# irconde/SSL4POLYP

Hardware: AMD Instinct MI355X
Metric: training-step images/sec/node, ViT-B/16 224^2 (cls fine-tune) (higher is better)
Workload: dtype bf16; 1 GPU; ViT-B/16 classification fine-tune, bs=64/GPU, 224^2, AdamW, random init, finetune mode full (finetune.py:49-91); global_batch=64, parallelism=dp1, launch=eager, lr_schedule=constant

## Files before the change

include/polypmae.h:

```cpp
#ifndef POLYPMAE_H
#define POLYPMAE_H
#include <stddef.h>
#include <stdint.h>

#ifdef __cplusplus
extern "C" {
#endif

enum pm_status { PM_OK = 0, PM_EINVAL = -1, PM_ESHAPE = -2, PM_EARCH = -3, PM_ELAUNCH = -4, PM_EALIGN = -5 };
enum pm_dtype { PM_F32 = 0, PM_BF16 = 1, PM_F16 = 2 };

enum pm_epilogue {
  PM_EPI_STORE = 0,
  PM_EPI_GELU = 1,
  PM_EPI_RESIDUAL = 2,
  PM_EPI_DGELU = 3,
  PM_EPI_ACCUM = 4
};

const char* pm_strerror(int status);
int pm_abi_version(void);

int pm_layernorm_fwd(const float* x, long ldx, const float* gamma, const float* beta, void* y, int out_dtype,
                     float* mean, float* rstd, int M, int D, float eps, void* stream);
// ... 21 lines not shown

#define PM_GEMM_GENERIC 0
#define PM_GEMM_LDS128 1
#define PM_GEMM_RING 2
#define PM_GEMM_RING_WGRAD 3
typedef struct pm_gemm_plan_info {
  int family;
  int cfg;
  int tile_m, tile_n;
  int split_k;
  int band;
  size_t ws_bytes;
} pm_gemm_plan_info;
int pm_gemm_plan(int a_kmajor, int b_kmajor, int in_dtype, int has_bias, int c_dtype, int ldc_is_n, int epilogue, int M, int N,
                 int K, size_t ws_bytes, const pm_gemm_opts* opts, pm_gemm_plan_info* info);

typedef struct pm_wgrad_item {
  const void* dY;
  long lddy;
  const void* X;
  long ldx;
  float* dW;
  long lddw;
  int n_out, n_in;
  int accumulate;
  float* dbias;
} pm_wgrad_item;
#define PM_GROUP_WHOLE_K (-1)
int pm_wgrad_group(const pm_wgrad_item* items, int n, int K, int in_dtype, int max_blocks, void* workspace, size_t ws_bytes,
                   void* stream);
// ... 253 lines not shown
```

ssl4polyp_amd/_lib.py:

```python
from __future__ import annotations

import ctypes
import os
from ctypes import c_char_p, c_float, c_int, c_long, c_void_p

PM_F32, PM_BF16, PM_F16 = 0, 1, 2
EPI_STORE, EPI_GELU, EPI_RESIDUAL, EPI_DGELU, EPI_ACCUM = 0, 1, 2, 3, 4

_HERE = os.path.dirname(os.path.abspath(__file__))
LIB_PATH = os.environ.get("POLYPMAE_LIB") or os.path.join(_HERE, "lib", "libpolypmae.so")

P, I, L, F = c_void_p, c_int, c_long, c_float

SIGNATURES = {
    "pm_layernorm_fwd": [P, L, P, P, P, I, P, P, I, I, F, P],
    "pm_layernorm_bwd": [P, I, P, L, P, P, P, P, L, P, L, P, I, P, P, P, I, I, P, ctypes.c_size_t, P],
    "pm_vit_block_fwd": [P, P],
    "pm_vit_block_bwd": [P, P],
    "pm_gemm": [P, L, I, P, L, I, I, P, P, L, I, I, P, P, I, I, I, P],
    "pm_gemm_ws": [P, L, I, P, L, I, I, P, P, L, I, I, P, P, I, I, I, P, ctypes.c_size_t, P],
    "pm_gemm_ex": [P, L, I, P, L, I, I, P, P, L, I, I, P, P, I, I, I, P, ctypes.c_size_t, P, P],
    "pm_wgrad_group": [P, I, I, I, I, P, ctypes.c_size_t, P],
    "pm_wgrad_group_plan": [P, I, I, I, P, P, P],
    "pm_gemm_plan": [I, I, I, I, I, I, I, I, I, I, ctypes.c_size_t, P, P],
    "pm_attention_plan": [I, I, I, I, I, I, P],
    "pm_attention_fwd": [P, P, P, I, I, I, I, I, P],
    "pm_attention_bwd": [P, P, P, P, P, P, I, I, I, I, I, P],
    "pm_colsum": [P, L, I, P, I, I, P],
    "pm_colsum_ws": [P, L, I, P, I, I, P, ctypes.c_size_t, P],
    "pm_patch_im2col": [P, P, P, L, I, I, I, I, I, I, P],
    "pm_pad_cast": [P, L, P, L, I, I, I, I, I, P],
    "pm_unpad_add": [P, L, P, L, I, I, I, P],
    "pm_assemble_tokens": [P, P, P, P, P, I, I, I, P],
    "pm_assemble_tokens_bwd": [P, P, P, I, P, P, I, I, I, P],
    "pm_mae_noise": [P, L, ctypes.c_ulonglong, ctypes.c_uint, P],
    "pm_mae_masking": [P, P, P, P, I, I, I, P],
    "pm_mae_unshuffle": [P, P, P, P, P, I, I, I, I, P],
    "pm_mae_unshuffle_bwd": [P, P, P, I, P, I, I, I, I, P, ctypes.c_size_t, P],
    "pm_mae_loss_fwd": [P, P, L, I, P, I, I, I, I, I, P],
# ... 161 lines not shown
```

ssl4polyp_amd/csrc/pm_common.h:

```cpp
#pragma once
#include <hip/hip_runtime.h>
#include <stdint.h>
#include "../../include/polypmae.h"

#ifdef PM_AUTO_VMCNT
#define PM_LDS_IMAGE
#else
#define PM_LDS_IMAGE __restrict__
#endif

#define PM_WAVE 64

typedef __attribute__((ext_vector_type(8))) __bf16 bf16x8;
typedef __attribute__((ext_vector_type(4))) __bf16 bf16x4;
typedef __attribute__((ext_vector_type(2))) __bf16 bf16x2;
typedef __attribute__((ext_vector_type(8))) _Float16 f16x8;
typedef __attribute__((ext_vector_type(4))) _Float16 f16x4;
typedef __attribute__((ext_vector_type(4))) short short4v;
typedef __attribute__((ext_vector_type(16))) float f32x16;
typedef __attribute__((ext_vector_type(4))) float f32x4;
typedef __attribute__((ext_vector_type(2))) float f32x2;
typedef __attribute__((ext_vector_type(4))) unsigned int u32x4;
typedef __attribute__((ext_vector_type(2))) unsigned int u32x2;

// ... 287 lines not shown
  }
#endif
  return gelu_erf4(v);
}
template <typename T> __device__ __forceinline__ f32x4 gelu_act_grad4(f32x4 v) {
#ifdef PM_GELU_POLY
  if constexpr (sizeof(T) == 2) {
    const f32x2 a = gelu_poly_grad2(f32x2{v[0], v[1]}), b = gelu_poly_grad2(f32x2{v[2], v[3]});
    return f32x4{a[0], a[1], b[0], b[1]};
  }
#endif
  return gelu_erf_grad4(v);
}
template <typename T> __device__ __forceinline__ f32x4 round_through(f32x4 v) {
  return f32x4{to_f32<T>(from_f32<T>(v[0])), to_f32<T>(from_f32<T>(v[1])), to_f32<T>(from_f32<T>(v[2])), to_f32<T>(from_f32<T>(v[3]))};
}

constexpr int kF0298 = 2446, kF0390 = 3196, kF0541 = 4433, kF0765 = 6270, kF0899 = 7373, kF1175 = 9633, kF1501 = 12299, kF1847 = 15137,
              kF1961 = 16069, kF2053 = 16819, kF2562 = 20995, kF3072 = 25172;
__device__ __forceinline__ int jdescale(int x, int n) { return (x + (1 << (n - 1))) >> n; }

__device__ __forceinline__ void jidct8(int* c, int s, bool first) {
  int z2 = c[2 * s], z3 = c[6 * s];
  int z1 = (z2 + z3) * kF0541;
  const int e2 = z1 + z3 * (-kF1847), e3 = z1 + z2 * kF0765;
  z2 = c[0];
  z3 = c[4 * s];
  const int e0 = (z2 + z3) << 13, e1 = (z2 - z3) << 13;
  const int t10 = e0 + e3, t13 = e0 - e3, t11 = e1 + e2, t12 = e1 - e2;
  int o0 = c[7 * s], o1 = c[5 * s], o2 = c[3 * s], o3 = c[s];
// ... 78 lines not shown
```

ssl4polyp_amd/csrc/pm_gemm.hip:

```cpp
#include "pm_common.h"
#include <type_traits>

namespace {

constexpr int BM = 128, BN = 128, KB = 128;
constexpr int TILE_BYTES = 128 * KB;
constexpr int kThreads = 256;
constexpr int STAGE_ROW = 64 * 4 + 16;
constexpr int STAGE_BYTES = 64 * STAGE_ROW;
constexpr int GLDS_LDS_BYTES = (4 * STAGE_BYTES > 4 * TILE_BYTES) ? 4 * STAGE_BYTES : 4 * TILE_BYTES;

struct GemmArgs {
  const void* X;
  const void* W;
  long ldx, ldw;
  const float* bias;
  void* C;
  long ldc;
  void* aux;
  const float* resid;
  int M, N, K;
  int epilogue;
  int c_dtype;
  int tiles_m, tiles_n;
  int split_k;
  int ksteps_split;
  float* xsum;
  int xsum_store;
  int col_major;
#ifdef PM_GEMM_STAMP
  unsigned long long* stamps;
#endif
};

#ifdef PM_GEMM_STAMP
#define PM_STAMP(i)                               \
  do {                                            \
    __builtin_amdgcn_sched_barrier(0);            \
    stamp_t[i] = __builtin_readcyclecounter();    \
    __builtin_amdgcn_sched_barrier(0);            \
  } while (0)
#else
#define PM_STAMP(i)
#endif
// ... 138 lines not shown
    } else if (epi == PM_EPI_DGELU) {
      const f32x4 pre = load4<T>(reinterpret_cast<const T*>(a.aux) + off);
      v *= gelu_act_grad4<T>(pre);
    }
    if (a.c_dtype == PM_F32) {
      store4<float>(reinterpret_cast<float*>(a.C) + off, v);
    } else if constexpr (sizeof(T) == 2) {
      store4<T>(reinterpret_cast<T*>(a.C) + off, v);
    } else {
      if (a.c_dtype == PM_F16) store4<_Float16>(reinterpret_cast<_Float16*>(a.C) + off, v);
      else store4<__bf16>(reinterpret_cast<__bf16*>(a.C) + off, v);
    }
  }
}

template <typename E, int NV>
__device__ __forceinline__ void epilogue_batch(const GemmArgs& a, int epi, const long (&off)[NV], const bool (&ok)[NV],
                                               f32x4 (&v)[NV]) {
  if (epi == PM_EPI_RESIDUAL || epi == PM_EPI_ACCUM) {
    const float* src = epi == PM_EPI_RESIDUAL ? a.resid : reinterpret_cast<const float*>(a.C);
    f32x4 r[NV];
#pragma unroll
    for (int e = 0; e < NV; ++e) r[e] = *reinterpret_cast<const f32x4*>(src + off[e]);
#pragma unroll
    for (int e = 0; e < NV; ++e)
      if (ok[e]) *reinterpret_cast<f32x4*>(reinterpret_cast<float*>(a.C) + off[e]) = r[e] + v[e];
    return;
  }
  if (epi == PM_EPI_DGELU) {
    f32x4 pre[NV];
#pragma unroll
    for (int e = 0; e < NV; ++e) pre[e] = load4<E>(reinterpret_cast<const E*>(a.aux) + off[e]);
#pragma unroll
    for (int e = 0; e < NV; ++e) v[e] *= gelu_act_grad4<E>(pre[e]);
  } else if (epi == PM_EPI_GELU) {
#pragma unroll
    for (int e = 0; e < NV; ++e) {
      if (a.aux && ok[e]) store4<E>(reinterpret_cast<E*>(a.aux) + off[e], v[e]);
      v[e] = gelu_act4<E>(round_through<E>(v[e]));
    }
  }
  if (a.c_dtype == PM_F32) {
#pragma unroll
    for (int e = 0; e < NV; ++e)
      if (ok[e]) store4<float>(reinterpret_cast<float*>(a.C) + off[e], v[e]);
  } else {
#pragma unroll
    for (int e = 0; e < NV; ++e)
      if (ok[e]) store4<E>(reinterpret_cast<E*>(a.C) + off[e], v[e]);
  }
}

template <typename E, int NV>
__device__ __forceinline__ void epilogue_batch8(const GemmArgs& a, int epi, const long (&off)[NV], const bool (&ok)[NV],
                                                f32x4 (&lo)[NV], f32x4 (&hi)[NV]) {
  if (epi == PM_EPI_DGELU) {
    f32x4 plo[NV], phi[NV];
#pragma unroll
    for (int u = 0; u < NV; ++u) load8_16<E>(reinterpret_cast<const E*>(a.aux) + off[u], plo[u], phi[u]);
#pragma unroll
    for (int u = 0; u < NV; ++u) {
      lo[u] *= gelu_act_grad4<E>(plo[u]);
      hi[u] *= gelu_act_grad4<E>(phi[u]);
    }
  } else if (epi == PM_EPI_GELU) {
#pragma unroll
    for (int u = 0; u < NV; ++u) {
      if (a.aux && ok[u]) store8_16<E>(reinterpret_cast<E*>(a.aux) + off[u], lo[u], hi[u]);
      lo[u] = gelu_act4<E>(round_through<E>(lo[u]));
      hi[u] = gelu_act4<E>(round_through<E>(hi[u]));
    }
  }
#pragma unroll
  for (int u = 0; u < NV; ++u)
    if (ok[u]) store8_16<E>(reinterpret_cast<E*>(a.C) + off[u], lo[u], hi[u]);
}

__device__ __forceinline__ void swap_halves(float& x, float& y) {
  typedef __attribute__((ext_vector_type(2))) unsigned u32x2;
  const u32x2 r = __builtin_amdgcn_permlane32_swap(__float_as_uint(x), __float_as_uint(y), false, false);
  x = __uint_as_float(r[0]);
  y = __uint_as_float(r[1]);
}

template <typename T, bool XK, bool WK>
// ... 237 lines not shown
  Frag16 f;
  f.u[0] = ((unsigned)(unsigned short)lo[0]) | (((unsigned)(unsigned short)lo[1]) << 16);
  f.u[1] = ((unsigned)(unsigned short)lo[2]) | (((unsigned)(unsigned short)lo[3]) << 16);
  f.u[2] = ((unsigned)(unsigned short)hi[0]) | (((unsigned)(unsigned short)hi[1]) << 16);
  f.u[3] = ((unsigned)(unsigned short)hi[2]) | (((unsigned)(unsigned short)hi[3]) << 16);
  return f;
}

template <int N> __device__ __forceinline__ void wait_vmcnt() {
  if constexpr (N == 0) asm volatile("s_waitcnt vmcnt(0)" ::: "memory");
  else if constexpr (N == 1) asm volatile("s_waitcnt vmcnt(1)" ::: "memory");
  else if constexpr (N == 2) asm volatile("s_waitcnt vmcnt(2)" ::: "memory");
  else if constexpr (N == 3) asm volatile("s_waitcnt vmcnt(3)" ::: "memory");
  else if constexpr (N == 4) asm volatile("s_waitcnt vmcnt(4)" ::: "memory");
  else if constexpr (N == 6) asm volatile("s_waitcnt vmcnt(6)" ::: "memory");
  else if constexpr (N == 8) asm volatile("s_waitcnt vmcnt(8)" ::: "memory");
  else if constexpr (N == 12) asm volatile("s_waitcnt vmcnt(12)" ::: "memory");
  else if constexpr (N == 16) asm volatile("s_waitcnt vmcnt(16)" ::: "memory");
  else if constexpr (N == 24) asm volatile("s_waitcnt vmcnt(24)" ::: "memory");
  else static_assert(N == 0, "add the immediate");
}

template <int BM_, int BN_, bool WK, bool DIRECT, bool PP, bool XK, bool XSUM, typename E>
__device__ __forceinline__ void gemm_v3_tile(GemmArgs& a, const int tile, const int split_idx) {
  constexpr int STAGES = V3_STAGES, NW = V3_WAVES;
  constexpr int WN = BN_ / 64, WM = NW / WN;
  constexpr int TM = BM_ / WM, TN = BN_ / WN;
  constexpr int MT = TM / 32, NTL = TN / 32;
  constexpr int XB = BM_ * 64, WB = BN_ * 64;
  constexpr int SB = XB + WB;
  constexpr int G = (SB / 1024 + NW - 1) / NW;
  static_assert((WB % (1024 * NW)) == 0 && ((XB % (1024 * NW)) == 0 || (!XK && XB == 12288 && DIRECT)),
                "whole wave-instructions per wave, except the 192-row k-normal X tile");
  extern __shared__ __attribute__((aligned(16))) char smem[];
  const int tid = threadIdx.x, lane = tid & 63;
  const int wave = __builtin_amdgcn_readfirstlane(tid >> 6);
  const int wm = wave / WN, wn = wave % WN;
#ifdef PM_GEMM_STAMP
  const unsigned long long stamp_entry = __builtin_readcyclecounter();
  const unsigned long long stamp_entry_rt = __builtin_amdgcn_s_memrealtime();
  unsigned long long stamp_loop_end = 0, stamp_loop_end_rt = 0;
  auto stamp_finish = [&]() {
    const unsigned long long t_issued = __builtin_readcyclecounter();
    asm volatile("s_waitcnt vmcnt(0)" ::: "memory");
    const unsigned long long t_acked = __builtin_readcyclecounter();
    if (a.stamps && lane == 0 && blockIdx.y == 0) {
      unsigned long long* o = a.stamps + ((long)blockIdx.x * NW + wave) * 16;
      o[8] = stamp_entry; o[9] = stamp_loop_end; o[10] = t_issued; o[11] = t_acked;
      o[12] = stamp_entry_rt; o[13] = stamp_loop_end_rt;
    }
  };
#endif
// ... 201 lines not shown
#endif
  } else {
    constexpr int DP = STAGES - 2;
    const int gq = wave >> 2;
#pragma unroll
    for (int t = 0; t < DP; ++t)
      if (t < nk) issue(t);
    constexpr bool UNEVEN = (XB % 8192) != 0;
    auto wait_one_stage_in_flight = [&]() {
      if constexpr (UNEVEN) {
        if (gq == 0) wait_vmcnt<G>(); else wait_vmcnt<G - 1>();
      } else {
        wait_vmcnt<G>();
      }
    };
    if (nk > 1) wait_one_stage_in_flight();
    else wait_vmcnt<0>();
    if (gq == 1) __builtin_amdgcn_s_barrier();
#ifdef PM_GEMM_STAMP
    unsigned long long stamp_t[8], stamp_acc[7] = {0, 0, 0, 0, 0, 0, 0};
#endif
    for (int t = 0; t < nk; ++t) {
      PM_STAMP(0);
      __builtin_amdgcn_s_barrier();
      PM_STAMP(1);
      Frag16 fw[2][NTL], fx[2][MT];
      read_frags(t, fw, fx);
      __builtin_amdgcn_sched_barrier(0);
      PM_STAMP(2);
      if (t + DP < nk) issue(t + DP);
      PM_STAMP(3);
      if (t + 2 < nk) wait_one_stage_in_flight();
      else wait_vmcnt<0>();
      PM_STAMP(4);
      asm volatile("s_waitcnt lgkmcnt(0)" ::: "memory");
      __builtin_amdgcn_sched_barrier(0);
      PM_STAMP(5);
      __builtin_amdgcn_s_barrier();
      PM_STAMP(6);
      mma_all(fw, fx);
#ifdef PM_GEMM_STAMP
      PM_STAMP(7);
#pragma unroll
      for (int i = 0; i < 7; ++i) stamp_acc[i] += stamp_t[i + 1] - stamp_t[i];
#endif
    }
#ifdef PM_GEMM_STAMP
    if (a.stamps && lane == 0 && blockIdx.y == 0) {
#pragma unroll
      for (int i = 0; i < 7; ++i) a.stamps[((long)blockIdx.x * NW + wave) * 16 + i] = stamp_acc[i];
      a.stamps[((long)blockIdx.x * NW + wave) * 16 + 7] = nk;
    }
#endif
    if (gq == 0) __builtin_amdgcn_s_barrier();
  }
#ifdef PM_GEMM_STAMP
  stamp_loop_end = __builtin_readcyclecounter();
  stamp_loop_end_rt = __builtin_amdgcn_s_memrealtime();
#endif
  if constexpr (XSUM) {
    if (do_xsum && lane < 16) {
#pragma unroll
      for (int j = 0; j < MT; ++j) {
        const int m = m0 + wm * TM + 32 * j + lane;
        if (m < a.M) a.xsum[m] = (a.xsum_store ? 0.f : a.xsum[m]) + xs[j][0];
        if (m + 16 < a.M) a.xsum[m + 16] = (a.xsum_store ? 0.f : a.xsum[m + 16]) + xs[j][1];
      }
    }
  }
  const int h = lane >> 5;
  const int epi = a.epilogue;
  if constexpr (DIRECT) {
    if (a.c_dtype != PM_F32 && epi != PM_EPI_RESIDUAL && epi != PM_EPI_ACCUM && (a.N & 7) == 0 && (a.ldc & 7) == 0) {
      constexpr int NV8 = NTL * 2;
      long noff8[NV8];
      bool nok8[NV8];
      f32x4 b0[NV8], b1[NV8];
#pragma unroll
      for (int i = 0; i < NTL; ++i)
#pragma unroll
        for (int p = 0; p < 2; ++p) {
          const int n = n0 + wn * TN + i * 32 + 16 * p + 8 * h;
          nok8[i * 2 + p] = n < a.N;
          noff8[i * 2 + p] = n < a.N ? n : a.N - 8;
        }
#pragma unroll
// ... 67 lines not shown
#pragma unroll
        for (int g = 0; g < 4; ++g) {
          const int e = i * 4 + g;
          off[g] = row + noff[e];
          ok[g] = mok && nok[e];
          v[g] = f32x4{acc[i][j][4 * g], acc[i][j][4 * g + 1], acc[i][j][4 * g + 2], acc[i][j][4 * g + 3]} + bv[e];
        }
        epilogue_batch<E, 4>(a, epi, off, ok, v);
      }
    }
#ifdef PM_GEMM_STAMP
    stamp_finish();
#endif
    return;
  }
  __syncthreads();
  char* st = smem + wave * V3_STAGE_WAVE;
#pragma unroll
  for (int mh = 0; mh < MT / 2; ++mh) {
#pragma unroll
    for (int nh = 0; nh < NTL / 2; ++nh) {
#pragma unroll
      for (int j = 0; j < 2; ++j) {
        const int ml = j * 32 + (lane & 31);
#pragma unroll
        for (int i = 0; i < 2; ++i)
#pragma unroll
          for (int g = 0; g < 4; ++g) {
            const f32x16& t16 = acc[nh * 2 + i][mh * 2 + j];
            const f32x4 v = {t16[4 * g], t16[4 * g + 1], t16[4 * g + 2], t16[4 * g + 3]};
// ... 13 lines not shown
        }
#pragma unroll
        for (int it4 = 0; it4 < 2; ++it4) {
          long off[4];
          bool ok[4];
          f32x4 lo[4], hi[4];
#pragma unroll
          for (int u = 0; u < 4; ++u) {
            const int ml = (it4 * 4 + u) * 8 + (lane >> 3);
            const int m = mw + ml;
            ok[u] = m < a.M && nok8;
            off[u] = (long)(m < a.M ? m : a.M - 1) * a.ldc + ncl8;
            lo[u] = *reinterpret_cast<const f32x4*>(st + ml * STAGE_ROW + c8 * 4) + b0;
            hi[u] = *reinterpret_cast<const f32x4*>(st + ml * STAGE_ROW + c8 * 4 + 16) + b1;
          }
          epilogue_batch8<E, 4>(a, epi, off, ok, lo, hi);
        }
        __builtin_amdgcn_wave_barrier();
        continue;
      }
      const int c4 = (lane & 15) * 4, n = nw + c4;
      const bool nok = n < a.N;
      const long ncl = nok ? n : a.N - 4;
      f32x4 bv = {0.f, 0.f, 0.f, 0.f};
      if (a.bias) bv = *reinterpret_cast<const f32x4*>(a.bias + ncl);
#pragma unroll
      for (int it4 = 0; it4 < 4; ++it4) {
        long off[4];
        bool ok[4];
        f32x4 v[4];
#pragma unroll
        for (int u = 0; u < 4; ++u) {
          const int ml = (it4 * 4 + u) * 4 + (lane >> 4);
          const int m = mw + ml;
          ok[u] = m < a.M && nok;
          off[u] = (long)(m < a.M ? m : a.M - 1) * a.ldc + ncl;
          v[u] = *reinterpret_cast<const f32x4*>(st + ml * STAGE_ROW + c4 * 4) + bv;
        }
        epilogue_batch<E, 4>(a, epi, off, ok, v);
      }
      __builtin_amdgcn_wave_barrier();
    }
  }
#ifdef PM_GEMM_STAMP
  stamp_finish();
#endif
}

template <int BM_, int BN_, bool WK, bool DIRECT, bool PP, bool XK, typename E>
__global__ __launch_bounds__(V3_WAVES * 64, 2) void gemm_v3_kernel(GemmArgs a) {
  gemm_v3_tile<BM_, BN_, WK, DIRECT, PP, XK, false, E>(a, xcd_remap(blockIdx.x, gridDim.x), blockIdx.y);
}

constexpr int kMaxGroup = 8;
struct WgradProb {
  const void* dY;
  const void* X;
  float* dW;
  long lddy, ldx, lddw;
  int M, N;
  int tiles_n, tiles_m;
  int tile_begin;
  int accumulate;
  float* dbias;
  float* slab;
  float* bias_part;
// ... 13 lines not shown
template <int BN_, typename E>
__global__ __launch_bounds__(V3_WAVES * 64, 2) void wgrad_group_kernel(WgradGroupArgs g) {
  const int work = g.total_tiles * g.split;
  for (int t = blockIdx.x; t < work; t += gridDim.x) {
    const int w = xcd_remap(t, work);
    const int slice = w / g.total_tiles, tile = w - slice * g.total_tiles;
    int pi = 0;
#pragma unroll
    for (int i = 1; i < kMaxGroup; ++i)
      if (i < g.n && tile >= g.p[i].tile_begin) pi = i;
    const WgradProb& pr = g.p[pi];
    GemmArgs a;
    a.X = pr.dY; a.W = pr.X; a.ldx = pr.lddy; a.ldw = pr.ldx; a.bias = nullptr; a.C = pr.dW; a.ldc = pr.lddw; a.aux = nullptr;
    a.resid = nullptr; a.M = pr.M; a.N = pr.N; a.K = g.K; a.epilogue = pr.accumulate ? PM_EPI_ACCUM : PM_EPI_STORE;
    a.c_dtype = PM_F32; a.tiles_m = pr.tiles_m; a.tiles_n = pr.tiles_n; a.split_k = 1; a.ksteps_split = 0;
    a.xsum = pr.dbias; a.xsum_store = 0;
    a.col_major = pr.tiles_m < pr.tiles_n;
    if (g.split > 1) {
      a.C = pr.slab; a.ldc = pr.N; a.epilogue = PM_EPI_STORE; a.split_k = g.split; a.ksteps_split = g.ksteps_split;
      a.xsum = pr.dbias ? pr.bias_part + (long)slice * pr.M : nullptr; a.xsum_store = 1;
    }
#ifdef PM_GEMM_STAMP
    a.stamps = g.stamps;
#endif
    gemm_v3_tile<256, BN_, true, true, true, true, true, E>(a, tile - pr.tile_begin, slice);
    __syncthreads();
  }
}

__global__ __launch_bounds__(256) void wgrad_group_reduce_kernel(WgradGroupArgs g) {
  const long stride = (long)gridDim.x * blockDim.x;
// ... 47 lines not shown
template <typename T>
int launch_glds(const GemmArgs& a, int xk, int wk, hipStream_t s) {
  return with_layouts(xk, wk, [&](auto XK, auto WK) {
    auto kern = gemm_glds_kernel<T, decltype(XK)::value, decltype(WK)::value>;
    PM_ALLOW_LDS(kern, GLDS_LDS_BYTES);
    hipLaunchKernelGGL(kern, dim3(a.tiles_m * a.tiles_n, a.split_k), dim3(kThreads), GLDS_LDS_BYTES, s, a);
    return pm_check_launch();
  });
}

template <typename E, int BM_, int BN_, bool WK, bool DIRECT, bool PP, bool XK>
int launch_v3(const GemmArgs& a, hipStream_t s) {
  constexpr int ring = V3_STAGES * (BM_ + BN_) * 64;
  constexpr int stage = DIRECT ? 0 : V3_WAVES * V3_STAGE_WAVE;
  constexpr size_t lds = ring > stage ? ring : stage;
  auto kern = gemm_v3_kernel<BM_, BN_, WK, DIRECT, PP, XK, E>;
  PM_ALLOW_LDS(kern, lds);
  hipLaunchKernelGGL(kern, dim3(a.tiles_m * a.tiles_n, a.split_k), dim3(V3_WAVES * 64), lds, s, a);
  return pm_check_launch();
}

struct RingCfg {
  int cfg;
  int bm;
  bool direct;
  bool pp;
  bool w_kmajor;
};
constexpr RingCfg kRingCfgs[] = {
    {8, 256, false, true, true},   {9, 256, true, true, false},   {10, 192, true, true, false},
// ... 5 lines not shown
    if (c.cfg == cfg && (!w_kmajor || c.w_kmajor)) return &c;
  return nullptr;
}

template <typename E, int I = 0>
int launch_ring(int cfg, const GemmArgs& a, int w_kmajor, hipStream_t s) {
  if constexpr (I == kNumRingCfgs) {
    return PM_EINVAL;
  } else {
    constexpr RingCfg c = kRingCfgs[I];
    if (c.cfg != cfg) return launch_ring<E, I + 1>(cfg, a, w_kmajor, s);
    if constexpr (c.w_kmajor)
      if (w_kmajor) return launch_v3<E, c.bm, 256, true, c.direct, c.pp, false>(a, s);
    return w_kmajor ? PM_EINVAL : launch_v3<E, c.bm, 256, false, c.direct, c.pp, false>(a, s);
  }
}

#ifdef PM_GEMM_STAMP
unsigned long long* g_stamps = nullptr;
#endif
inline bool is16(int dtype) { return dtype == PM_BF16 || dtype == PM_F16; }

int launch_splitk_reduce(const void* slabs, void* out, long ldc, int M, int N, int splits, bool accumulate, hipStream_t s) {
  const long nvec = (long)M * (N >> 2);
  int grid = (int)((nvec + 255) / 256);
  if (grid > 2048) grid = 2048;
  hipLaunchKernelGGL(splitk_reduce_kernel, dim3(grid), dim3(256), 0, s, (const float*)slabs, (float*)out, ldc, M, N, splits,
                     accumulate ? 1 : 0);
  return pm_check_launch();
}
// ... 111 lines not shown
  const int epc = is16(in_dtype) ? 8 : 4;
  if ((lda % epc) || (ldb % epc) || (ldc & 3)) return PM_EALIGN;
  if (((uintptr_t)A & 15) || ((uintptr_t)B & 15) || ((uintptr_t)C & 15)) return PM_EALIGN;
  if (epilogue == PM_EPI_DGELU && !aux) return PM_EINVAL;
  if (epilogue == PM_EPI_RESIDUAL && !resid) return PM_EINVAL;
  GemmArgs a;
  a.X = A; a.W = B; a.ldx = lda; a.ldw = ldb; a.bias = bias; a.C = C; a.ldc = ldc; a.aux = aux; a.resid = resid;
  a.M = M; a.N = N; a.K = K; a.epilogue = epilogue; a.c_dtype = c_dtype;
  a.tiles_m = (M + p.tile_m - 1) / p.tile_m;
  a.tiles_n = (N + p.tile_n - 1) / p.tile_n;
  a.split_k = p.split_k;
  a.ksteps_split = p.ksteps_split;
  a.xsum = nullptr;
  a.xsum_store = 0;
  a.col_major = p.band;
#ifdef PM_GEMM_STAMP
  a.stamps = g_stamps;
#endif
  if (p.split_k > 1) {
    a.C = workspace;
    a.epilogue = PM_EPI_STORE;
  }
  hipStream_t s = pm_stream(stream);
  int st = PM_EINVAL;
  switch (p.family) {
    case PM_GEMM_GENERIC: PM_DISPATCH_ACT(in_dtype, T, st = launch_generic<T>(a, a_kmajor, b_kmajor, s)); break;
    case PM_GEMM_LDS128: PM_DISPATCH_ACT(in_dtype, T, st = launch_glds<T>(a, a_kmajor, b_kmajor, s)); break;
    case PM_GEMM_RING: PM_DISPATCH_16(in_dtype, E, st = launch_ring<E>(p.cfg, a, b_kmajor, s)); break;
    case PM_GEMM_RING_WGRAD:
      PM_DISPATCH_16(in_dtype, E, st = p.tile_n == 128 ? launch_v3<E, 256, 128, true, true, true, true>(a, s)
// ... 8 lines not shown

extern "C" int pm_gemm_plan(int a_kmajor, int b_kmajor, int in_dtype, int has_bias, int c_dtype, int ldc_is_n, int epilogue, int M,
                            int N, int K, size_t ws_bytes, const pm_gemm_opts* opts, pm_gemm_plan_info* info) {
  const GemmPlan p = plan_gemm(a_kmajor, b_kmajor, in_dtype, has_bias != 0, c_dtype, ldc_is_n != 0, epilogue, M, N, K, ws_bytes > 0,
                               ws_bytes, opts);
  if (p.status == PM_OK && info)
    *info = pm_gemm_plan_info{p.family, p.cfg, p.tile_m, p.tile_n, p.split_k, p.band, p.ws_bytes};
  return p.status;
}

extern "C" size_t pm_gemm_workspace_bytes(int a_kmajor, int b_kmajor, int in_dtype, int M, int N, int K,
                                          const pm_gemm_opts* opts) {
  if (!(a_kmajor && b_kmajor)) return 0;
  const GemmPlan p = plan_gemm(a_kmajor, b_kmajor, in_dtype, false, PM_F32, true, PM_EPI_STORE, M, N, K, true, (size_t)-1, opts);
  return p.status == PM_OK ? p.ws_bytes : 0;
}

#ifdef PM_GEMM_STAMP
extern "C" void pm_debug_gemm_stamps(void* p) { g_stamps = reinterpret_cast<unsigned long long*>(p); }
#endif

extern "C" int pm_gemm_ex(const void* A, long lda, int a_kmajor, const void* B, long ldb, int b_kmajor, int in_dtype,
                          const float* bias, void* C, long ldc, int c_dtype, int epilogue, void* aux, const float* resid,
                          int M, int N, int K, void* workspace, size_t ws_bytes, const pm_gemm_opts* opts, void* stream) {
  return gemm_dispatch(A, lda, a_kmajor, B, ldb, b_kmajor, in_dtype, bias, C, ldc, c_dtype, epilogue, aux, resid, M, N, K,
                       workspace, ws_bytes, opts, stream);
}

extern "C" int pm_gemm_ws(const void* A, long lda, int a_kmajor, const void* B, long ldb, int b_kmajor, int in_dtype,
                          const float* bias, void* C, long ldc, int c_dtype, int epilogue, void* aux,
// ... 158 lines not shown
```

ssl4polyp_amd/engine.py:

```python
from __future__ import annotations

from dataclasses import dataclass
from typing import Callable, Dict, List, Optional, Sequence, Tuple

import contextlib
import ctypes
import os

import torch

from . import _lib
from ._lib import EPI_ACCUM, EPI_DGELU, EPI_GELU, EPI_RESIDUAL, EPI_STORE, PM_BF16, PM_F16, PM_F32

LN_EPS = 1e-6

BLOCK_PARAM_NAMES = (
    "norm1.weight", "norm1.bias", "attn.qkv.weight", "attn.qkv.bias", "attn.proj.weight", "attn.proj.bias",
    "norm2.weight", "norm2.bias", "mlp.fc1.weight", "mlp.fc1.bias", "mlp.fc2.weight", "mlp.fc2.bias")


def _ptr(t: Optional[torch.Tensor]) -> Optional[int]:
    return None if t is None else t.data_ptr()


# ... 33 lines not shown
            buf = self.bufs[key] = torch.empty(max(nbytes, self.FLOOR), dtype=torch.uint8, device=device)
            self.generation += 1
        return buf


_STREAMS: Dict[Tuple[int, str], "torch.cuda.Stream"] = {}


def _shared_stream(device, role: str):
    dev = torch.device(device)
    key = (dev.index if dev.index is not None else torch.cuda.current_device(), role)
    st = _STREAMS.get(key)
    if st is None:
        st = _STREAMS[key] = torch.cuda.Stream(device=dev)
    return st


def reserve_streams(device) -> None:
    dev = torch.device(device)
    torch.zeros(1, device=dev)
    for role in ("aux0", "side"):
        with torch.cuda.stream(_shared_stream(dev, role)):
            torch.zeros(1, device=dev)
    torch.cuda.synchronize(dev)


PRECISIONS = {"bf16": (torch.bfloat16, PM_BF16), "fp16": (torch.float16, PM_F16), "fp32": (torch.float32, PM_F32)}


class Kernels:
# ... 623 lines not shown
```

ssl4polyp_amd/models.py:

```python
from __future__ import annotations

import math
from functools import partial
from typing import Dict, List, Optional

import numpy as np
import torch
import torch.nn as nn

from . import _lib
from .engine import (BLOCK_PARAM_NAMES, EPI_STORE, BlockStack, Kernels, StackGeom, StackWorkspace, _ptr, _stream)
from .flat import FlatParams

_DEFAULT_PRECISION = "bf16"


def get_1d_sincos_pos_embed_from_grid(embed_dim, pos):
    assert embed_dim % 2 == 0
    omega = np.arange(embed_dim // 2, dtype=np.float64)
    omega /= embed_dim / 2.0
    omega = 1.0 / 10000 ** omega
    out = np.einsum("m,d->md", pos.reshape(-1), omega)
    return np.concatenate([np.sin(out), np.cos(out)], axis=1)


def get_2d_sincos_pos_embed(embed_dim, grid_size, cls_token=False):
# ... 75 lines not shown

    def block_end(self, prefix: str, i: int) -> int:
        f = self.flat
        j = f.index[f"{prefix}{i}.mlp.fc2.weight"]
        return f.offset[j] + f.numel[j]

    def ensure(self, device: torch.device) -> None:
        if device.type != "cuda":
            raise _lib.PolypMaeError("ssl4polyp_amd models run on the MI355X HIP path only (got a CPU tensor); "
                                     "there is no eager fallback")
        if self.k is None:
            self.k = Kernels(self.precision, self.eps)
        if self.flat is None or set(self.flat.names) != {n for n, _ in self.module.named_parameters()}:
            self.flat = FlatParams(self.module, self.k.act_dtype)
        if not self.flat.bound(device):
            self.flat.materialize(device)
            self.pool.clear()
            self._wcache = {}
        if self.flat.shadow_stale():
            self.wait_updates()
            self.k.cast(self.flat.P["mat"], self.flat.S)
            self.flat.mark_shadow_fresh()
        if self.pending_updates:
            f = self.flat
            self.wait_updates(mat_through=f.offset[f.index["blocks.0.attn.qkv.weight"]])

    def stack_weights(self, prefix: str, depth: int):
        hit = self._wcache.get(prefix)
        if hit is not None:
            return hit
# ... 727 lines not shown
```

Measured before the change: 6526 images/sec.

## Use LDS-resident bf16 lookup tables for GELU and dGELU in GEMM epilogues

Precomputes GELU and GELU-gradient values for every bf16 input across a bounded exponent range into a device table. The 256x256 ping-pong bf16 GEMM copies this table into spare LDS during the last k-steps, overlapping the copy with the main loop. Its epilogue then looks values up instead of evaluating erf-based math, with a wave-wide fallback to direct computation for out-of-range inputs. This removes transcendental ALU work from the FC1 and dGELU epilogues, at the cost of more LDS per block, extra loads at the K tail, and a new kernel variant.

```diff
diff --git a/include/polypmae.h b/include/polypmae.h
--- a/include/polypmae.h
+++ b/include/polypmae.h
@@ -59,6 +59,10 @@
 } pm_gemm_plan_info;
 int pm_gemm_plan(int a_kmajor, int b_kmajor, int in_dtype, int has_bias, int c_dtype, int ldc_is_n, int epilogue, int M, int N,
                  int K, size_t ws_bytes, const pm_gemm_opts* opts, pm_gemm_plan_info* info);
+
+int pm_gelu_tables_init(int device);
+int pm_gelu_table_index(int bits16);
+int pm_gelu_table_bytes(void);
 
 typedef struct pm_wgrad_item {
   const void* dY;
diff --git a/ssl4polyp_amd/_lib.py b/ssl4polyp_amd/_lib.py
--- a/ssl4polyp_amd/_lib.py
+++ b/ssl4polyp_amd/_lib.py
@@ -23,6 +23,9 @@
     "pm_wgrad_group": [P, I, I, I, I, P, ctypes.c_size_t, P],
     "pm_wgrad_group_plan": [P, I, I, I, P, P, P],
     "pm_gemm_plan": [I, I, I, I, I, I, I, I, I, I, ctypes.c_size_t, P, P],
+    "pm_gelu_tables_init": [I],
+    "pm_gelu_table_index": [I],
+    "pm_gelu_table_bytes": [],
     "pm_attention_plan": [I, I, I, I, I, I, P],
     "pm_attention_fwd": [P, P, P, I, I, I, I, I, P],
     "pm_attention_bwd": [P, P, P, P, P, P, I, I, I, I, I, P],
diff --git a/ssl4polyp_amd/csrc/pm_common.h b/ssl4polyp_amd/csrc/pm_common.h
--- a/ssl4polyp_amd/csrc/pm_common.h
+++ b/ssl4polyp_amd/csrc/pm_common.h
@@ -325,6 +325,20 @@
 }
 template <typename T> __device__ __forceinline__ f32x4 round_through(f32x4 v) {
   return f32x4{to_f32<T>(from_f32<T>(v[0])), to_f32<T>(from_f32<T>(v[1])), to_f32<T>(from_f32<T>(v[2])), to_f32<T>(from_f32<T>(v[3]))};
+}
+
+constexpr int kGeluTabExpLo = 111, kGeluTabExps = 20;
+constexpr int kGeluTabHalf = kGeluTabExps * 128;
+constexpr int kGeluTabSlots = 2 * kGeluTabHalf;
+constexpr int kGeluTabBytes = 24576;
+__host__ __device__ inline unsigned gelu_tab_slot(unsigned bits, unsigned& a) {
+  a = (bits & 0x7FFFu) - (unsigned)(kGeluTabExpLo << 7);
+  return a + ((bits >> 15) & 1u) * (unsigned)kGeluTabHalf;
+}
+__host__ __device__ inline int gelu_tab_index(unsigned bits) {
+  unsigned a;
+  const unsigned s = gelu_tab_slot(bits & 0xFFFFu, a);
+  return a < (unsigned)kGeluTabHalf ? (int)s : -1;
 }
 
 constexpr int kF0298 = 2446, kF0390 = 3196, kF0541 = 4433, kF0765 = 6270, kF0899 = 7373, kF1175 = 9633, kF1501 = 12299, kF1847 = 15137,
diff --git a/ssl4polyp_amd/csrc/pm_gemm.hip b/ssl4polyp_amd/csrc/pm_gemm.hip
--- a/ssl4polyp_amd/csrc/pm_gemm.hip
+++ b/ssl4polyp_amd/csrc/pm_gemm.hip
@@ -1,4 +1,6 @@
 #include "pm_common.h"
+#include <atomic>
+#include <mutex>
 #include <type_traits>
 
 namespace {
@@ -28,6 +30,7 @@
   float* xsum;
   int xsum_store;
   int col_major;
+  const float* act_table;
 #ifdef PM_GEMM_STAMP
   unsigned long long* stamps;
 #endif
@@ -196,9 +199,33 @@
   }
 }
 
-template <typename E, int NV>
+template <typename E, bool GRAD, int NV>
+__device__ __forceinline__ void gelu_from_table(const float* tab, const f32x4 (&x)[NV], f32x4 (&out)[NV]) {
+  unsigned worst = 0;
+#pragma unroll
+  for (int u = 0; u < NV; ++u)
+#pragma unroll
+    for (int k = 0; k < 4; ++k) {
+      unsigned a;
+      const unsigned s = gelu_tab_slot(__float_as_uint(x[u][k]) >> 16, a);
+      worst = a > worst ? a : worst;
+      const unsigned ac = a < (unsigned)kGeluTabHalf ? a : (unsigned)kGeluTabHalf - 1;
+      out[u][k] = tab[s - a + ac];
+    }
+  if (__builtin_amdgcn_ballot_w64(worst >= (unsigned)kGeluTabHalf) != 0) {
+#pragma unroll
+    for (int u = 0; u < NV; ++u) {
+      const f32x4 c = GRAD ? gelu_act_grad4<E>(x[u]) : gelu_act4<E>(x[u]);
+#pragma unroll
+      for (int k = 0; k < 4; ++k) out[u][k] = gelu_tab_index(__float_as_uint(x[u][k]) >> 16) >= 0 ? out[u][k] : c[k];
+      __builtin_amdgcn_sched_barrier(0);
+    }
+  }
+}
+
+template <typename E, int NV, bool TAB = false>
 __device__ __forceinline__ void epilogue_batch(const GemmArgs& a, int epi, const long (&off)[NV], const bool (&ok)[NV],
-                                               f32x4 (&v)[NV]) {
+                                               f32x4 (&v)[NV], const float* tab = nullptr) {
   if (epi == PM_EPI_RESIDUAL || epi == PM_EPI_ACCUM) {
     const float* src = epi == PM_EPI_RESIDUAL ? a.resid : reinterpret_cast<const float*>(a.C);
     f32x4 r[NV];
@@ -213,13 +240,30 @@
     f32x4 pre[NV];
 #pragma unroll
     for (int e = 0; e < NV; ++e) pre[e] = load4<E>(reinterpret_cast<const E*>(a.aux) + off[e]);
-#pragma unroll
-    for (int e = 0; e < NV; ++e) v[e] *= gelu_act_grad4<E>(pre[e]);
+    if constexpr (TAB) {
+      f32x4 g[NV];
+      gelu_from_table<E, true, NV>(tab, pre, g);
+#pragma unroll
+      for (int e = 0; e < NV; ++e) v[e] *= g[e];
+    } else {
+#pragma unroll
+      for (int e = 0; e < NV; ++e) v[e] *= gelu_act_grad4<E>(pre[e]);
+    }
   } else if (epi == PM_EPI_GELU) {
-#pragma unroll
-    for (int e = 0; e < NV; ++e) {
-      if (a.aux && ok[e]) store4<E>(reinterpret_cast<E*>(a.aux) + off[e], v[e]);
-      v[e] = gelu_act4<E>(round_through<E>(v[e]));
+    if constexpr (TAB) {
+      f32x4 r[NV];
+#pragma unroll
+      for (int e = 0; e < NV; ++e) {
+        if (a.aux && ok[e]) store4<E>(reinterpret_cast<E*>(a.aux) + off[e], v[e]);
+        r[e] = round_through<E>(v[e]);
+      }
+      gelu_from_table<E, false, NV>(tab, r, v);
+    } else {
+#pragma unroll
+      for (int e = 0; e < NV; ++e) {
+        if (a.aux && ok[e]) store4<E>(reinterpret_cast<E*>(a.aux) + off[e], v[e]);
+        v[e] = gelu_act4<E>(round_through<E>(v[e]));
+      }
     }
   }
   if (a.c_dtype == PM_F32) {
@@ -233,24 +277,47 @@
   }
 }
 
-template <typename E, int NV>
+template <typename E, int NV, bool TAB = false>
 __device__ __forceinline__ void epilogue_batch8(const GemmArgs& a, int epi, const long (&off)[NV], const bool (&ok)[NV],
-                                                f32x4 (&lo)[NV], f32x4 (&hi)[NV]) {
+                                                f32x4 (&lo)[NV], f32x4 (&hi)[NV], const float* tab = nullptr) {
   if (epi == PM_EPI_DGELU) {
     f32x4 plo[NV], phi[NV];
 #pragma unroll
     for (int u = 0; u < NV; ++u) load8_16<E>(reinterpret_cast<const E*>(a.aux) + off[u], plo[u], phi[u]);
-#pragma unroll
-    for (int u = 0; u < NV; ++u) {
-      lo[u] *= gelu_act_grad4<E>(plo[u]);
-      hi[u] *= gelu_act_grad4<E>(phi[u]);
+    if constexpr (TAB) {
+      f32x4 g[NV];
+      gelu_from_table<E, true, NV>(tab, plo, g);
+#pragma unroll
+      for (int u = 0; u < NV; ++u) lo[u] *= g[u];
+      gelu_from_table<E, true, NV>(tab, phi, g);
+#pragma unroll
+      for (int u = 0; u < NV; ++u) hi[u] *= g[u];
+    } else {
+#pragma unroll
+      for (int u = 0; u < NV; ++u) {
+        lo[u] *= gelu_act_grad4<E>(plo[u]);
+        hi[u] *= gelu_act_grad4<E>(phi[u]);
+      }
     }
   } else if (epi == PM_EPI_GELU) {
-#pragma unroll
-    for (int u = 0; u < NV; ++u) {
-      if (a.aux && ok[u]) store8_16<E>(reinterpret_cast<E*>(a.aux) + off[u], lo[u], hi[u]);
-      lo[u] = gelu_act4<E>(round_through<E>(lo[u]));
-      hi[u] = gelu_act4<E>(round_through<E>(hi[u]));
+    if constexpr (TAB) {
+      f32x4 x[NV];
+#pragma unroll
+      for (int u = 0; u < NV; ++u) {
+        if (a.aux && ok[u]) store8_16<E>(reinterpret_cast<E*>(a.aux) + off[u], lo[u], hi[u]);
+        x[u] = round_through<E>(lo[u]);
+      }
+      gelu_from_table<E, false, NV>(tab, x, lo);
+#pragma unroll
+      for (int u = 0; u < NV; ++u) x[u] = round_through<E>(hi[u]);
+      gelu_from_table<E, false, NV>(tab, x, hi);
+    } else {
+#pragma unroll
+      for (int u = 0; u < NV; ++u) {
+        if (a.aux && ok[u]) store8_16<E>(reinterpret_cast<E*>(a.aux) + off[u], lo[u], hi[u]);
+        lo[u] = gelu_act4<E>(round_through<E>(lo[u]));
+        hi[u] = gelu_act4<E>(round_through<E>(hi[u]));
+      }
     }
   }
 #pragma unroll
@@ -518,6 +585,7 @@
   else if constexpr (N == 3) asm volatile("s_waitcnt vmcnt(3)" ::: "memory");
   else if constexpr (N == 4) asm volatile("s_waitcnt vmcnt(4)" ::: "memory");
   else if constexpr (N == 6) asm volatile("s_waitcnt vmcnt(6)" ::: "memory");
+  else if constexpr (N == 7) asm volatile("s_waitcnt vmcnt(7)" ::: "memory");
   else if constexpr (N == 8) asm volatile("s_waitcnt vmcnt(8)" ::: "memory");
   else if constexpr (N == 12) asm volatile("s_waitcnt vmcnt(12)" ::: "memory");
   else if constexpr (N == 16) asm volatile("s_waitcnt vmcnt(16)" ::: "memory");
@@ -525,7 +593,7 @@
   else static_assert(N == 0, "add the immediate");
 }
 
-template <int BM_, int BN_, bool WK, bool DIRECT, bool PP, bool XK, bool XSUM, typename E>
+template <int BM_, int BN_, bool WK, bool DIRECT, bool PP, bool XK, bool XSUM, typename E, bool TAB = false, int EPI_C = -1>
 __device__ __forceinline__ void gemm_v3_tile(GemmArgs& a, const int tile, const int split_idx) {
   constexpr int STAGES = V3_STAGES, NW = V3_WAVES;
   constexpr int WN = BN_ / 64, WM = NW / WN;
@@ -540,6 +608,20 @@
   const int tid = threadIdx.x, lane = tid & 63;
   const int wave = __builtin_amdgcn_readfirstlane(tid >> 6);
   const int wm = wave / WN, wn = wave % WN;
+  static_assert(!TAB || (!DIRECT && PP && !XK && !XSUM && BM_ == 256 && BN_ == 256 && std::is_same<E, __bf16>::value),
+                "the table form exists for the bf16 ping-pong kernel with the staged epilogue");
+  constexpr int kTabAt = NW * V3_STAGE_WAVE, kTabPieces = kGeluTabBytes / 1024 / NW;
+  static_assert(kTabAt >= STAGES * SB || !TAB, "the table copy must not overlap a ring slot");
+  static_assert(kTabPieces * 1024 * NW == kGeluTabBytes && kTabAt + kGeluTabBytes <= 160 * 1024, "whole pieces per wave, inside the LDS");
+  constexpr bool use_tab = TAB;
+  [[maybe_unused]] const float* tab = reinterpret_cast<const float*>(smem + kTabAt);
+  [[maybe_unused]] auto issue_table = [&]() {
+#pragma unroll
+    for (int i = 0; i < kTabPieces; ++i) {
+      const int j = wave + NW * i;
+      glds16(reinterpret_cast<const char*>(a.act_table) + 1024 * j + 16 * lane, smem + kTabAt + 1024 * j);
+    }
+  };
 #ifdef PM_GEMM_STAMP
   const unsigned long long stamp_entry = __builtin_readcyclecounter();
   const unsigned long long stamp_entry_rt = __builtin_amdgcn_s_memrealtime();
@@ -771,13 +853,27 @@
         wait_vmcnt<G>();
       }
     };
-    if (nk > 1) wait_one_stage_in_flight();
-    else wait_vmcnt<0>();
+    bool tab_flying = false;
+    auto wait_stage = [&](bool next_flying) {
+      if constexpr (TAB) {
+        if (tab_flying) {
+          if (next_flying) wait_vmcnt<G + kTabPieces>(); else wait_vmcnt<kTabPieces>();
+          return;
+        }
+      }
+      if (next_flying) wait_one_stage_in_flight(); else wait_vmcnt<0>();
+    };
+    if (use_tab && nk <= DP) {
+      issue_table();
+      tab_flying = true;
+    }
+    wait_stage(nk > 1);
     if (gq == 1) __builtin_amdgcn_s_barrier();
 #ifdef PM_GEMM_STAMP
     unsigned long long stamp_t[8], stamp_acc[7] = {0, 0, 0, 0, 0, 0, 0};
 #endif
-    for (int t = 0; t < nk; ++t) {
+    auto kstep = [&](int t, auto tail) {
+      constexpr bool TAIL = decltype(tail)::value;
       PM_STAMP(0);
       __builtin_amdgcn_s_barrier();
       PM_STAMP(1);
@@ -786,9 +882,19 @@
       __builtin_amdgcn_sched_barrier(0);
       PM_STAMP(2);
       if (t + DP < nk) issue(t + DP);
+      if constexpr (TAIL) {
+        if (t + DP == nk - 1) {
+          issue_table();
+          tab_flying = true;
+        }
+      }
       PM_STAMP(3);
-      if (t + 2 < nk) wait_one_stage_in_flight();
-      else wait_vmcnt<0>();
+      if constexpr (TAIL) {
+        wait_stage(t + 2 < nk);
+      } else {
+        if (t + 2 < nk) wait_one_stage_in_flight();
+        else wait_vmcnt<0>();
+      }
       PM_STAMP(4);
       asm volatile("s_waitcnt lgkmcnt(0)" ::: "memory");
       __builtin_amdgcn_sched_barrier(0);
@@ -801,6 +907,12 @@
 #pragma unroll
       for (int i = 0; i < 7; ++i) stamp_acc[i] += stamp_t[i + 1] - stamp_t[i];
 #endif
+    };
+    const int nk_plain = use_tab ? (nk > DP + 1 ? nk - (DP + 1) : 0) : nk;
+    int t = 0;
+    for (; t < nk_plain; ++t) kstep(t, std::false_type{});
+    if constexpr (TAB) {
+      for (; t < nk; ++t) kstep(t, std::true_type{});
     }
 #ifdef PM_GEMM_STAMP
     if (a.stamps && lane == 0 && blockIdx.y == 0) {
@@ -826,7 +938,7 @@
     }
   }
   const int h = lane >> 5;
-  const int epi = a.epilogue;
+  const int epi = EPI_C >= 0 ? EPI_C : a.epilogue;
   if constexpr (DIRECT) {
     if (a.c_dtype != PM_F32 && epi != PM_EPI_RESIDUAL && epi != PM_EPI_ACCUM && (a.N & 7) == 0 && (a.ldc & 7) == 0) {
       constexpr int NV8 = NTL * 2;
@@ -924,6 +1036,9 @@
 #endif
     return;
   }
+  if constexpr (TAB) {
+    if (use_tab) wait_vmcnt<0>();
+  }
   __syncthreads();
   char* st = smem + wave * V3_STAGE_WAVE;
 #pragma unroll
@@ -967,7 +1082,7 @@
             lo[u] = *reinterpret_cast<const f32x4*>(st + ml * STAGE_ROW + c8 * 4) + b0;
             hi[u] = *reinterpret_cast<const f32x4*>(st + ml * STAGE_ROW + c8 * 4 + 16) + b1;
           }
-          epilogue_batch8<E, 4>(a, epi, off, ok, lo, hi);
+          epilogue_batch8<E, 4, TAB>(a, epi, off, ok, lo, hi, tab);
         }
         __builtin_amdgcn_wave_barrier();
         continue;
@@ -990,7 +1105,7 @@
           off[u] = (long)(m < a.M ? m : a.M - 1) * a.ldc + ncl;
           v[u] = *reinterpret_cast<const f32x4*>(st + ml * STAGE_ROW + c4 * 4) + bv;
         }
-        epilogue_batch<E, 4>(a, epi, off, ok, v);
+        epilogue_batch<E, 4, TAB>(a, epi, off, ok, v, tab);
       }
       __builtin_amdgcn_wave_barrier();
     }
@@ -1003,6 +1118,10 @@
 template <int BM_, int BN_, bool WK, bool DIRECT, bool PP, bool XK, typename E>
 __global__ __launch_bounds__(V3_WAVES * 64, 2) void gemm_v3_kernel(GemmArgs a) {
   gemm_v3_tile<BM_, BN_, WK, DIRECT, PP, XK, false, E>(a, xcd_remap(blockIdx.x, gridDim.x), blockIdx.y);
+}
+template <bool WK, int EPI>
+__global__ __launch_bounds__(V3_WAVES * 64, 2) void gemm_v3_table_kernel(GemmArgs a) {
+  gemm_v3_tile<256, 256, WK, false, true, false, false, __bf16, true, EPI>(a, xcd_remap(blockIdx.x, gridDim.x), blockIdx.y);
 }
 
 constexpr int kMaxGroup = 8;
@@ -1046,7 +1165,7 @@
     a.X = pr.dY; a.W = pr.X; a.ldx = pr.lddy; a.ldw = pr.ldx; a.bias = nullptr; a.C = pr.dW; a.ldc = pr.lddw; a.aux = nullptr;
     a.resid = nullptr; a.M = pr.M; a.N = pr.N; a.K = g.K; a.epilogue = pr.accumulate ? PM_EPI_ACCUM : PM_EPI_STORE;
     a.c_dtype = PM_F32; a.tiles_m = pr.tiles_m; a.tiles_n = pr.tiles_n; a.split_k = 1; a.ksteps_split = 0;
-    a.xsum = pr.dbias; a.xsum_store = 0;
+    a.xsum = pr.dbias; a.xsum_store = 0; a.act_table = nullptr;
     a.col_major = pr.tiles_m < pr.tiles_n;
     if (g.split > 1) {
       a.C = pr.slab; a.ldc = pr.N; a.epilogue = PM_EPI_STORE; a.split_k = g.split; a.ksteps_split = g.ksteps_split;
@@ -1124,6 +1243,16 @@
   constexpr int ring = V3_STAGES * (BM_ + BN_) * 64;
   constexpr int stage = DIRECT ? 0 : V3_WAVES * V3_STAGE_WAVE;
   constexpr size_t lds = ring > stage ? ring : stage;
+  if constexpr (std::is_same<E, __bf16>::value && BM_ == 256 && BN_ == 256 && !DIRECT && PP && !XK) {
+    if (a.act_table) {
+      auto go = [&](auto tkern) {
+        PM_ALLOW_LDS(tkern, lds + kGeluTabBytes);
+        hipLaunchKernelGGL(tkern, dim3(a.tiles_m * a.tiles_n, a.split_k), dim3(V3_WAVES * 64), lds + kGeluTabBytes, s, a);
+        return pm_check_launch();
+      };
+      return a.epilogue == PM_EPI_DGELU ? go(gemm_v3_table_kernel<WK, PM_EPI_DGELU>) : go(gemm_v3_table_kernel<WK, PM_EPI_GELU>);
+    }
+  }
   auto kern = gemm_v3_kernel<BM_, BN_, WK, DIRECT, PP, XK, E>;
   PM_ALLOW_LDS(kern, lds);
   hipLaunchKernelGGL(kern, dim3(a.tiles_m * a.tiles_n, a.split_k), dim3(V3_WAVES * 64), lds, s, a);
@@ -1159,6 +1288,31 @@
       if (w_kmajor) return launch_v3<E, c.bm, 256, true, c.direct, c.pp, false>(a, s);
     return w_kmajor ? PM_EINVAL : launch_v3<E, c.bm, 256, false, c.direct, c.pp, false>(a, s);
   }
+}
+
+__global__ __launch_bounds__(256) void gelu_tables_fill_kernel(float* __restrict__ gelu, float* __restrict__ dgelu) {
+  const unsigned b0 = (blockIdx.x * 256 + threadIdx.x) * 4;
+  if (b0 >= 65536u || gelu_tab_index(b0) < 0) return;
+  const f32x4 x = {bf16_bits_to_f32(b0), bf16_bits_to_f32(b0 + 1), bf16_bits_to_f32(b0 + 2), bf16_bits_to_f32(b0 + 3)};
+  const f32x4 g = gelu_act4<__bf16>(x), d = gelu_act_grad4<__bf16>(x);
+#pragma unroll
+  for (int k = 0; k < 4; ++k) {
+    const int i = gelu_tab_index(b0 + k);
+    gelu[i] = g[k];
+    dgelu[i] = d[k];
+  }
+}
+
+constexpr int kMaxTableDevices = 64;
+std::atomic<const float*> g_gelu_tables[kMaxTableDevices];
+std::mutex g_gelu_tables_mu;
+
+const float* gelu_table(int epilogue) {
+  int dev = -1;
+  if (hipGetDevice(&dev) != hipSuccess || dev < 0 || dev >= kMaxTableDevices) return nullptr;
+  const float* t = g_gelu_tables[dev].load(std::memory_order_acquire);
+  if (!t) return nullptr;
+  return epilogue == PM_EPI_DGELU ? t + kGeluTabBytes / sizeof(float) : t;
 }
 
 #ifdef PM_GEMM_STAMP
@@ -1300,6 +1454,9 @@
   a.xsum = nullptr;
   a.xsum_store = 0;
   a.col_major = p.band;
+  a.act_table = nullptr;
+  if (p.family == PM_GEMM_RING && p.cfg == 8 && in_dtype == PM_BF16 && (epilogue == PM_EPI_GELU || epilogue == PM_EPI_DGELU))
+    a.act_table = gelu_table(epilogue);
 #ifdef PM_GEMM_STAMP
   a.stamps = g_stamps;
 #endif
@@ -1338,6 +1495,31 @@
   if (!(a_kmajor && b_kmajor)) return 0;
   const GemmPlan p = plan_gemm(a_kmajor, b_kmajor, in_dtype, false, PM_F32, true, PM_EPI_STORE, M, N, K, true, (size_t)-1, opts);
   return p.status == PM_OK ? p.ws_bytes : 0;
+}
+
+extern "C" int pm_gelu_table_index(int bits16) { return gelu_tab_index((unsigned)bits16 & 0xFFFFu); }
+extern "C" int pm_gelu_table_bytes(void) { return kGeluTabBytes; }
+
+extern "C" int pm_gelu_tables_init(int device) {
+  if (device < 0 || device >= kMaxTableDevices) return PM_EINVAL;
+  std::lock_guard<std::mutex> lock(g_gelu_tables_mu);
+  if (g_gelu_tables[device].load(std::memory_order_acquire)) return PM_OK;
+  int prev = -1;
+  if (hipGetDevice(&prev) != hipSuccess) return PM_ELAUNCH;
+  if (prev != device && hipSetDevice(device) != hipSuccess) return PM_EINVAL;
+  float* buf = nullptr;
+  int st = PM_OK;
+  if (hipMalloc(reinterpret_cast<void**>(&buf), 2 * kGeluTabBytes) != hipSuccess) st = PM_ELAUNCH;
+  if (st == PM_OK && hipMemset(buf, 0, 2 * kGeluTabBytes) != hipSuccess) st = PM_ELAUNCH;
+  if (st == PM_OK) {
+    hipLaunchKernelGGL(gelu_tables_fill_kernel, dim3(65536 / 4 / 256), dim3(256), 0, nullptr, buf, buf + kGeluTabBytes / sizeof(float));
+    st = pm_check_launch();
+  }
+  if (st == PM_OK && hipDeviceSynchronize() != hipSuccess) st = PM_ELAUNCH;
+  if (st == PM_OK) g_gelu_tables[device].store(buf, std::memory_order_release);
+  else if (buf) (void)hipFree(buf);
+  if (prev != device) (void)hipSetDevice(prev);
+  return st;
 }
 
 #ifdef PM_GEMM_STAMP
diff --git a/ssl4polyp_amd/engine.py b/ssl4polyp_amd/engine.py
--- a/ssl4polyp_amd/engine.py
+++ b/ssl4polyp_amd/engine.py
@@ -71,6 +71,17 @@
     if st is None:
         st = _STREAMS[key] = torch.cuda.Stream(device=dev)
     return st
+
+
+_DEVICE_STATE: set = set()
+
+
+def init_device(device) -> None:
+    dev = torch.device(device)
+    idx = dev.index if dev.index is not None else torch.cuda.current_device()
+    if idx not in _DEVICE_STATE:
+        _lib.check(_lib.load().pm_gelu_tables_init(idx), "pm_gelu_tables_init")
+        _DEVICE_STATE.add(idx)
 
 
 def reserve_streams(device) -> None:
diff --git a/ssl4polyp_amd/models.py b/ssl4polyp_amd/models.py
--- a/ssl4polyp_amd/models.py
+++ b/ssl4polyp_amd/models.py
@@ -9,7 +9,7 @@
 import torch.nn as nn
 
 from . import _lib
-from .engine import (BLOCK_PARAM_NAMES, EPI_STORE, BlockStack, Kernels, StackGeom, StackWorkspace, _ptr, _stream)
+from .engine import (BLOCK_PARAM_NAMES, EPI_STORE, BlockStack, Kernels, StackGeom, StackWorkspace, _ptr, _stream, init_device)
 from .flat import FlatParams
 
 _DEFAULT_PRECISION = "bf16"
@@ -115,6 +115,7 @@
         if self.flat is None or set(self.flat.names) != {n for n, _ in self.module.named_parameters()}:
             self.flat = FlatParams(self.module, self.k.act_dtype)
         if not self.flat.bound(device):
+            init_device(device)
             self.flat.materialize(device)
             self.pool.clear()
             self._wcache = {}
```

After: 6584 images/sec, median of 6. No clear change (+0.9%).
